# da03/torch-Attention-OCR

Measured on AMD Instinct MI355X. Metric: image-lines/sec (train step), higher is better.
Workload: dtype bf16; 1 GPU; c3: 32x256 crops, batch 256/GPU, VGG-7 + BiLSTM(256) + 2-layer attn decoder, L=24; global_batch=256, per_gpu_batch=256, img=32x256, decoder_steps=24, parallelism=dp1, input_feed=True

## Files before the change

### torch-attention-ocr_amd/csrc/knobs.h

```cpp
#pragma once
#include <cstdlib>

namespace aocr { namespace knob {
#define AOCR_KNOB_SET(FN, NAME, DEF)  inline bool FN() { return std::getenv(NAME) != nullptr; }
#define AOCR_KNOB_ON(FN, NAME, DEF)   inline bool FN() { const char* e = std::getenv(NAME); return e && e[0] == '1'; }
#define AOCR_KNOB_NOT0(FN, NAME, DEF) inline bool FN() { const char* e = std::getenv(NAME); return !(e && e[0] == '0'); }
#define AOCR_KNOB_INT(FN, NAME, DEF)  inline int FN() { const char* e = std::getenv(NAME); return e ? std::atoi(e) : (DEF); }
#define AOCR_KNOB_RAW(FN, NAME, DEF)  inline const char* FN() { return std::getenv(NAME); }
#define KNOB(NAME, KIND, DEF, EFFECT) AOCR_KNOB_##KIND(NAME, #NAME, DEF)
#define KNOB_CLAMP(NAME, KIND, DEF, LO, HI, EFFECT) inline int NAME() { const char* e = std::getenv(#NAME); if (!e) return (DEF); const int n = std::atoi(e); return n < (LO) ? (LO) : n > (HI) ? (HI) : n; }
#define KNOB_ALSO(FN, NAME, KIND, DEF, EFFECT) AOCR_KNOB_##KIND(FN, #NAME, DEF)

KNOB(AOCR_TRACE,                 SET,  0,    "one stderr line per launch decision of the traced launchers")
KNOB(AOCR_PROBE,                 SET,  0,    "aocr_profile_kernel prints the in-kernel clock probe of the tagged conv launch")
KNOB(AOCR_PROBE_LAYER,           RAW,  0,    "3|4|5: aocr_profile_kernel id 0 replays that conv layer's tagged forward launch instead of conv6's")
KNOB(AOCR_DBG_STOP,              INT,  0,    "1|2: stop the CNN backward pass at that stage and leave its gradient map in place (tap g0)")
KNOB_ALSO(AOCR_DBG_STOP_SET, AOCR_DBG_STOP, SET, 0, "cnn_wgrad_on_side: any value keeps the CNN filter gradients off the side stream")
KNOB(AOCR_DC_STAMPS,             RAW,  0,    "cycle stamps of the decoder cluster / chain kernels (stamps build); a value starting with b: beam launches only")
KNOB(AOCR_SEQ_STAMP,             SET,  0,    "cycle stamps of the whole-sequence encoder forward kernel")
KNOB(AOCR_SEQ_ABL,               INT,  0,    "timing-only ablation bits of the whole-sequence encoder forward kernel")
KNOB(AOCR_CL_REMOTE,             SET,  0,    "cluster kernels exchange through write-through stores as if their members were not on one XCD")
KNOB(AOCR_NO_DMA,                ON,   0,    "no LDS-DMA kernels at all (the 128 x 128 LDS kernels)")
KNOB(AOCR_FORCE_DMA,             ON,   0,    "LDS-DMA kernels wherever their shape constraints hold, however the grid fills the chip")
KNOB(AOCR_NO_HALO,               ON,   0,    "no halo-resident 3 x 3 kernel (the im2col LDS-DMA kernel)")
KNOB(AOCR_HALO8,                 SET,  0,    "the 8-wave gemm_halo_bf16_kernel instead of the 4-wave gemm_halo4_bf16_kernel")
KNOB(AOCR_HALO4_STAGED,          INT,  7,    "bits: output tiles of the 256 x 256 kernels through LDS -- 1 fp32 data gradient, 2 fp32 conv forward, 4 pooled")
KNOB(AOCR_NO_NARROW_WIDE,        SET,  0,    "conv7 forward on 128 x 128 tiles instead of 256 x 128 tiles of the narrow LDS-DMA kernel")
KNOB(AOCR_NO_NARROW_STAGED,      ON,   0,    "quad epilogue of the narrow LDS-DMA kernel instead of the staged tile")
KNOB(AOCR_NO_DMA128,             ON,   0,    "128 x 128 tiles on the register-staged kernel instead of gemm_dma128_kernel")
KNOB(AOCR_DMA128_W4,             ON,   0,    "gemm_dma128_kernel's 4-wave form at every grid size")
KNOB(AOCR_NO_HH_NARROW,          SET,  0,    "hoisted bf16 GEMMs on the 128 x 128 kernels instead of the narrow LDS-DMA kernel")
KNOB(AOCR_HH_NARROW_FULL_ONLY,   ON,   0,    "hoisted GEMMs take the narrow LDS-DMA kernel only when M is whole 256-row tiles")
KNOB(AOCR_NO_HH_CAT,             ON,   0,    "the encoder's d X as two products instead of one over the concatenated K range")
KNOB(AOCR_NO_SKINNY,             SET,  0,    "128 x 128 tiles for skinny products (N <= 64) instead of the step kernel; also turns project_loss_kernel off")
KNOB(AOCR_NO_PROJ_FUSE,          ON,   0,    "projector, criterion and projector data gradient as three launches instead of project_loss_kernel")
KNOB(AOCR_NO_BN_STATS_FUSE,      SET,  0,    "BatchNorm statistics of conv3 / conv5 by a pass over y instead of from the conv epilogue")
KNOB(AOCR_BN_Y16,                SET,  0,    "pre-BatchNorm maps stored as bf16 (outside the parity tolerance)")
KNOB(AOCR_DX16,                  ON,   0,    "bf16 data-gradient maps for the BatchNorm backward / un-pool passes (outside the parity tolerance)")
KNOB(AOCR_BNB_FUSE,              ON,   0,    "BatchNorm backward's sums pass from the data gradient's staged fp32 tile (measured slower)")
KNOB(AOCR_WGRAD_ATOMIC,          SET,  0,    "split-K filter gradients through fp32 atomics instead of slabs + splitk_reduce_kernel")
KNOB(AOCR_NO_WGRAD_HALO,         ON,   0,    "filter gradients on the one-tap-per-tile kernels instead of conv_wgrad_halo_kernel")
KNOB(AOCR_WGRAD_HALO_MINN,       INT,  576,  "smallest N = 9 Cin that takes conv_wgrad_halo_kernel (conv2 upwards)")
KNOB(AOCR_WGRAD_HALO_MINSTEPS,   INT,  0,    "> 0: at small P fewer, longer k ranges of at least n steps instead of a full round of the chip")
KNOB(AOCR_WGRAD_HALO_RAGGED,     NOT0, 1,    "0: conv_wgrad_halo_kernel only for rows of whole 32-pixel segments")
KNOB(AOCR_NO_WGRAD_ISSUE_MID,    ON,   0,    "conv_wgrad_halo_kernel issues the next DMA pieces before its first MFMA instead of between the k-halves")
KNOB(AOCR_NO_WGRAD_DMA_GROUPED,  ON,   0,    "recurrent weight gradients on wgrad_tr_grouped_kernel instead of wgrad_dma_grouped_kernel")
KNOB(AOCR_WGRAD_DMA_WGS,         INT,  256,  "workgroups wgrad_dma_grouped_kernel aims at per launch (one round)")
KNOB(AOCR_WGRAD_DMA_MINK,        INT,  2048, "smallest K (rows L B / T B) that takes wgrad_dma_grouped_kernel")
KNOB(AOCR_NO_LDS_F32,            SET,  0,    "fragment-from-global fp32 GEMM instead of the LDS-tiled kernels")
KNOB(AOCR_NO_F32T,               ON,   0,    "gemm_lds_f32_kernel instead of gemm_f32t_kernel")
KNOB(AOCR_F32T_TILE,             INT,  0,    "1|2|3: force gemm_f32t_kernel's tile (128 x 128 / 64 x 128 / 64 x 64)")
KNOB(AOCR_NO_F32W,               ON,   0,    "fragment-from-global kernel instead of gemm_f32w_kernel")
KNOB_CLAMP(AOCR_F32W_MINK,       INT,  192,  32, 0x7fffffff, "least K per k range of gemm_f32w_kernel's split (at least 32)")
KNOB(AOCR_NO_STEP_F32,           ON,   0,    "gemm_small_kernel<false> instead of gemm_step_f32_kernel")
KNOB(AOCR_STEP_F32_W16,          ON,   0,    "gemm_step_f32_kernel's 16-wave form for deep K on small grids (measured slower)")
KNOB(AOCR_NO_QUARTER_TILES,      SET,  0,    "full gate tiles instead of 8-unit tiles at small batch (fp32 mode)")
KNOB(AOCR_NO_HALF_TILES,         ON,   0,    "32-unit gate tiles instead of half gate tiles on small grids")
KNOB(AOCR_HALF_TILES_MAXGRID,    INT,  200,  "the 32-unit grid size below which gate products take half tiles")
KNOB(AOCR_STEP_WAVES4,           SET,  0,    "4-wave gemm_step_kernel instead of 8 waves")
KNOB(AOCR_STEP_WAVES16,          SET,  0,    "16 waves for plain step products at K >= 1024 (measured slower)")
KNOB(AOCR_NO_STEP_MT2,           ON,   0,    "one 32-row tile per workgroup instead of two where the grid allows")
KNOB(AOCR_STEP_MT2_MINK,         INT,  2048, "the K from which one plain product takes two row tiles per workgroup")
KNOB(AOCR_NO_STEPL,              ON,   0,    "step products on gemm_step_kernel instead of stepl.h")
KNOB(AOCR_STEPL_MIN_WGS,         INT,  -1,   ">= 0: stepl.h from n of its own workgroups whatever the kind of launch")
KNOB(AOCR_BIG_STEP,              ON,   0,    "step products as 128 x 128 LDS-DMA tiles + an elementwise cell pass (measured slower)")
KNOB(AOCR_BIG_STEP_MIN_ROWS,     INT,  320,  "rows from which AOCR_BIG_STEP applies")
KNOB(AOCR_CONV1_SCALAR,          SET,  0,    "conv1's filter gradient on the scalar kernel instead of the packed one")
KNOB(AOCR_UNPOOL4,               SET,  0,    "un-pool on the 4-channel kernels instead of unpool8_kernel")
KNOB(AOCR_BN_PARTIAL_OLD,        SET,  0,    "4-byte-access BatchNorm partial sums instead of bn_partial4_kernel")
KNOB(AOCR_ATTN_BWD_TWO_PASS,     SET,  0,    "the streamed attention backward kernel in two passes over the context instead of one")
KNOB(AOCR_NO_ATTN_BF16,          SET,  0,    "fp32-context attention instead of the bf16-context kernels")
KNOB(AOCR_NO_ATTN_BEAM_GROUP,    SET,  0,    "beam decode at T > 64 with one attention workgroup per hypothesis instead of per image")
KNOB(AOCR_ATTN_NW16,             SET,  0,    "16-wave attention at T <= 32, Hd = 1024")
KNOB(AOCR_NO_CHAIN_CTXA,         SET,  0,    "the Hd = 1024 chain with a q = W_a h launch per step instead of scores against ctx W_a")
KNOB(AOCR_NO_BN_FOLD,            SET,  0,    "unfused evaluation-mode BatchNorm")
KNOB(AOCR_NO_SIDE_WGRAD,         SET,  0,    "no side stream: weight gradients on the main stream")
KNOB(AOCR_SIDE_PLAIN,            SET,  0,    "side stream at normal priority")
KNOB(AOCR_NO_SIDE_PROLOGUE,      ON,   0,    "gradient zeroing / weight shadows / token table on the main stream in front of conv1")
KNOB(AOCR_NO_SHADOW_SPLIT,       ON,   0,    "conv2 waits for the whole shadow table instead of its own taps")
KNOB(AOCR_NO_CNN_WGRAD_SIDE,     ON,   0,    "the CNN's filter gradients on the main stream")
KNOB(AOCR_CNN_WGRAD_AFTER_DGRAD, ON,   0,    "filter gradient of a stage started behind its data gradient (slower)")
KNOB(AOCR_NO_COLSUM_DEFER,       SET,  0,    "one column-sum launch per bias instead of two deferred ones")
KNOB(AOCR_CONV1_RECOMPUTE,       SET,  0,    "conv1's filter gradient re-evaluates the layer instead of reading the forward pass's routes")
KNOB(AOCR_NO_SEQ,                ON,   0,    "encoder: no whole-sequence kernels at all (per-step launches)")
KNOB(AOCR_NO_CLUSTER,            ON,   0,    "encoder: no cluster kernels (one-workgroup-per-16-rows whole-sequence kernels)")
KNOB(AOCR_NO_LAYER_PIPE,         SET,  0,    "stacked encoder layer after layer instead of the chunk wavefront")
KNOB(AOCR_LAYER_PIPE_CHUNKS,     RAW,  0,    "n: force the wavefront's chunk count")
KNOB(AOCR_ENC_DC_COPY,           ON,   0,    "split copy of the decoder's initial-state gradient in front of the encoder BPTT")
KNOB(AOCR_NO_ENC_WGRAD_SIDE,     ON,   0,    "the encoder's weight gradients on the main stream")
KNOB(AOCR_SIDE_GO_LATE,          ON,   0,    "side streams released behind d(context) instead of behind the decoder BPTT")
KNOB(AOCR_NO_SIDE2,              ON,   0,    "no second side stream")
KNOB(AOCR_JOIN_BEFORE_CNN_BWD,   ON,   0,    "the main stream joins the side stream in front of the CNN backward pass")
KNOB(AOCR_NO_Q_SIDE,             ON,   0,    "q of all steps on the main stream")
KNOB(AOCR_NO_EMB_TABLE,          ON,   0,    "first decoder layer's embedding part as a gathered tensor + product instead of the per-token table")
KNOB(AOCR_NO_EMB_TABLE_CHAIN,    ON,   0,    "the launch chain's first decoder layer without the per-token table")
KNOB(AOCR_NO_DEC_CLUSTER,        ON,   0,    "decoder: launch chain instead of the cluster kernels")
KNOB(AOCR_NO_DEC_CLUSTER_BWD,    ON,   0,    "decoder BPTT: launch chain instead of the cluster kernel")
KNOB(AOCR_NO_DEC_CLUSTER_DROP,   SET,  0,    "decoder under dropout: launch chain instead of the cluster kernels")
KNOB(AOCR_NO_DEC_GREEDY,         SET,  0,    "greedy decode on the launch chain instead of the cluster kernel")
KNOB(AOCR_NO_DECODE_SHADOWS,     ON,   0,    "the decode launch chain without bf16 shadows of its beam state")
KNOB(AOCR_NO_DEC_CHAINS,         ON,   0,    "dec_cluster.hip's one-chain kernels instead of dec_chain.hip")
KNOB(AOCR_NO_DEC_CHAINS_BWD,     SET,  0,    "the same for the decoder BPTT only")
KNOB(AOCR_NO_DEC_CHAINS_GREEDY,  SET,  0,    "the same for greedy decode only")
KNOB(AOCR_NO_DEC_CHAINS_BEAM,    SET,  0,    "beam search on the per-step launch chain")
KNOB(AOCR_CH_NO_RES,             SET,  0,    "the ctx W_a tile re-read per step instead of resident (T <= 64)")
KNOB(AOCR_NO_DEC_EARLY,          SET,  0,    "no early exit of the greedy kernel")
KNOB(AOCR_ENC_RT2,               ON,   0,    "two row tiles per encoder group although one fits the chip")
KNOB(AOCR_ENC_RH16,              ON,   0,    "encoder forward on 16-row groups")
KNOB(AOCR_ENC_BWD_RH,            RAW,  0,    "8|16: force 8- / 16-row groups in the encoder BPTT")
KNOB(AOCR_ONE_COMM,              SET,  0,    "SyncBN on the gradient communicator (no ncclCommSplit)")
KNOB(AOCR_COMM_EARLY_BUCKET0,    ON,   0,    "release gradient bucket 0 before the encoder BPTT")
KNOB_CLAMP(AOCR_COMM_RESERVE_CUS, INT, 32,   0, 128, "compute units the encoder cluster launches then leave to the collective (0..128)")

#undef KNOB_ALSO
#undef KNOB_CLAMP
#undef KNOB
#undef AOCR_KNOB_RAW
#undef AOCR_KNOB_INT
#undef AOCR_KNOB_NOT0
#undef AOCR_KNOB_ON
#undef AOCR_KNOB_SET

}}
```

### torch-attention-ocr_amd/csrc/mfma_gemm.h

```cpp
#pragma once
#include <hip/hip_runtime.h>
#include <stdint.h>
#include <type_traits>
#include <utility>

namespace aocr {

typedef float f32x16 __attribute__((ext_vector_type(16)));
typedef float f32x4 __attribute__((ext_vector_type(4)));
typedef __bf16 bf16x8 __attribute__((ext_vector_type(8)));

template <int NV> struct Frag { float v[NV]; };

template <bool BF16> struct Mode {
  static constexpr int NV = BF16 ? 8 : 4;
  static constexpr int CHUNK = BF16 ? 16 : 8;
};


struct LoadK {
  const float* p0; int64_t ld0; int K0;
  const float* p1; int64_t ld1;
  int rows; int K; int vec;
  struct Ctx { const float* b0; const float* b1; bool ok; };
// ... 1946 lines not shown
#pragma unroll
  for (int i = 0; i < 4; ++i)
#pragma unroll
    for (int j = 0; j < 2; ++j)
#pragma unroll
      for (int e = 0; e < 16; ++e) acc[i][j][e] = 0.f;

  const int g = lane >> 4, q = (lane >> 2) & 3, p4 = lane & 3;
  const unsigned rowoff = (8 * h + q) * 512 + (16 * (g & 1) + 4 * p4) * 2;
  unsigned aseg[4], bseg[2];
#pragma unroll
  for (int i = 0; i < 4; ++i) aseg[i] = rowoff + (((wm * 4 + i) ^ q) << 6);
#pragma unroll
  for (int i = 0; i < 2; ++i) bseg[i] = 16384 + rowoff + (((wn * 2 + i) ^ q) << 6);

  typedef unsigned long long u64;
  typedef u64 u64x2 __attribute__((ext_vector_type(2)));
  const unsigned lbase = (unsigned)(uintptr_t)((__attribute__((address_space(3))) unsigned char*)lds);
#define AOCR_TRR(dst, addr, OFF) asm volatile("ds_read_b64_tr_b16 %0, %1 offset:" #OFF : "=v"(dst) : "v"(addr))
#pragma unroll
  for (int t = 0; t < 3; ++t) issue();
  for (int kt = 0; kt < nk; ++kt) {
    asm volatile("s_waitcnt vmcnt(8)" ::: "memory");
    __builtin_amdgcn_s_barrier();
    const unsigned sl = lbase + (kt & 3) * 32768;
    u64 fa[2][4][2], fb[2][2][2];
#pragma unroll
    for (int i = 0; i < 4; ++i) {
      const unsigned ad = sl + aseg[i];
      if constexpr (ABL & 4) { fa[0][i][0] = fa[0][i][1] = fa[1][i][0] = fa[1][i][1] = ad; continue; }
      AOCR_TRR(fa[0][i][0], ad, 0); AOCR_TRR(fa[0][i][1], ad, 2048); AOCR_TRR(fa[1][i][0], ad, 8192); AOCR_TRR(fa[1][i][1], ad, 10240);
    }
#pragma unroll
    for (int i = 0; i < 2; ++i) {
      const unsigned ad = sl + bseg[i];
      if constexpr (ABL & 4) { fb[0][i][0] = fb[0][i][1] = fb[1][i][0] = fb[1][i][1] = ad; continue; }
      AOCR_TRR(fb[0][i][0], ad, 0); AOCR_TRR(fb[0][i][1], ad, 2048); AOCR_TRR(fb[1][i][0], ad, 8192); AOCR_TRR(fb[1][i][1], ad, 10240);
    }
    if constexpr (!(ABL & 1)) issue();
    asm volatile("s_waitcnt lgkmcnt(0)"
                 : "+v"(fa[0][0][0]), "+v"(fa[0][0][1]), "+v"(fa[0][1][0]), "+v"(fa[0][1][1]), "+v"(fa[0][2][0]), "+v"(fa[0][2][1]),
                   "+v"(fa[0][3][0]), "+v"(fa[0][3][1]), "+v"(fb[0][0][0]), "+v"(fb[0][0][1]), "+v"(fb[0][1][0]), "+v"(fb[0][1][1])
                 :: "memory");
    asm volatile(""
                 : "+v"(fa[1][0][0]), "+v"(fa[1][0][1]), "+v"(fa[1][1][0]), "+v"(fa[1][1][1]), "+v"(fa[1][2][0]), "+v"(fa[1][2][1]),
                   "+v"(fa[1][3][0]), "+v"(fa[1][3][1]), "+v"(fb[1][0][0]), "+v"(fb[1][0][1]), "+v"(fb[1][1][0]), "+v"(fb[1][1][1])
                 :: "memory");
#pragma unroll
    for (int s2 = 0; s2 < 2; ++s2)
#pragma unroll
      for (int mi = 0; mi < 4; ++mi)
#pragma unroll
        for (int ni = 0; ni < 2; ++ni) {
          const u64x2 av = {fa[s2][mi][0], fa[s2][mi][1]}, bv = {fb[s2][ni][0], fb[s2][ni][1]};
          if constexpr (ABL & 2) { acc[mi][ni][0] += (float)(unsigned)(av[0] ^ bv[1]); continue; }
          acc[mi][ni] = __builtin_amdgcn_mfma_f32_32x32x16_bf16(__builtin_bit_cast(bf16x8, av), __builtin_bit_cast(bf16x8, bv), acc[mi][ni], 0, 0, 0);
        }
  }
#undef AOCR_TRR
  asm volatile("s_waitcnt vmcnt(0) lgkmcnt(0)" ::: "memory");
  const int r = lane & 31;
  const int m0 = m_blk + wm * 128, n0 = n_blk + wn * 64;
  if constexpr (std::is_same<EP, EpStore>::value && ABL == 0) {
    if (part && !ep.flags && !ep.bias && !ep.bias2 && !ep.C1 && !ep.Cb && !ep.dg && m_blk + 256 <= ep.M && n_blk + 256 <= ep.N) {
      tile256_store_f32<2, 512>(ep.C, ep.ldc, nullptr, false, acc, lds, m_blk, n_blk, wm, wn, r, h, tid);
      return;
    }
  }
#pragma unroll
  for (int mi = 0; mi < 4; ++mi)
#pragma unroll
    for (int qq = 0; qq < 4; ++qq) {
      float v[2][4];
#pragma unroll
      for (int ni = 0; ni < 2; ++ni)
#pragma unroll
        for (int i = 0; i < 4; ++i) v[ni][i] = acc[mi][ni][4 * qq + i];
      ep.template quad<2>(m0 + 32 * mi + 8 * qq + 4 * h, n0 + r, 32, v);
    }
}

struct WgDmaProblem { const bf16_t* A; const bf16_t* B; long long lda, ldb; int M, N, K, gx, tiles, ks, kper, first; float* part; float* C; long long ldc; long long f4first; };
struct WgDmaArgs { int n, total; long long f4total; WgDmaProblem p[8]; };
template <int UNUSED = 0>
__global__ __launch_bounds__(512, 1) void wgrad_dma_grouped_kernel(WgDmaArgs g, const bf16_t* zero) {
  __shared__ __attribute__((aligned(1024))) unsigned char lds[4 * 32768];
  int pi = 0;
#pragma unroll
  for (int i = 1; i < 8; ++i) if (i < g.n && (int)blockIdx.x >= g.p[i].first) pi = i;
  const WgDmaProblem& P = g.p[pi];
  const int local = blockIdx.x - P.first;
  const int zsp = local / P.tiles, bid = local - zsp * P.tiles;
  const int m_blk = (bid / P.gx) * 256, n_blk = (bid % P.gx) * 256;
  const int kbeg = zsp * P.kper, kend = min(P.K, kbeg + P.kper);
  const int nk = kend > kbeg ? (kend - kbeg + 31) >> 5 : 0;
  const int tid = threadIdx.x, lane = tid & 63, wave = __builtin_amdgcn_readfirstlane(tid >> 6);
  const int h = lane >> 5, wm = wave >> 2, wn = wave & 3;
  const bf16_t* pa[2]; const bf16_t* pb[2]; int ka[2];
#pragma unroll
  for (int j = 0; j < 2; ++j) {
    const int krow = 2 * (2 * wave + j) + (lane >> 5), pos = lane & 31;
    const int chunk = ((((pos >> 2) ^ (krow & 3)) << 2) | (pos & 3));
    ka[j] = kbeg + krow;
    pa[j] = P.A + (long long)ka[j] * P.lda + m_blk + 8 * chunk; pb[j] = P.B + (long long)ka[j] * P.ldb + n_blk + 8 * chunk;
  }
  const long long astep = 32 * P.lda, bstep = 32 * P.ldb;
  unsigned char* const wbase = lds + (2 * wave) * 1024;
  int slot = 0;
  auto issue = [&]() {
#pragma unroll
    for (int j = 0; j < 2; ++j) { dma16(dma_select(ka[j] < kend, pa[j], zero), wbase + slot * 32768 + j * 1024); pa[j] += astep; }
#pragma unroll
    for (int j = 0; j < 2; ++j) { dma16(dma_select(ka[j] < kend, pb[j], zero), wbase + slot * 32768 + 16384 + j * 1024); pb[j] += bstep; ka[j] += 32; }
    slot = (slot + 1) & 3;
  };
  f32x16 acc[4][2];
#pragma unroll
  for (int i = 0; i < 4; ++i)
#pragma unroll
    for (int j = 0; j < 2; ++j)
#pragma unroll
      for (int e = 0; e < 16; ++e) acc[i][j][e] = 0.f;
  const int gq = lane >> 4, q = (lane >> 2) & 3, p4 = lane & 3;
  const unsigned rowoff = (8 * h + q) * 512 + (16 * (gq & 1) + 4 * p4) * 2;
  unsigned aseg[4], bseg[2];
#pragma unroll
  for (int i = 0; i < 4; ++i) aseg[i] = rowoff + (((wm * 4 + i) ^ q) << 6);
#pragma unroll
  for (int i = 0; i < 2; ++i) bseg[i] = 16384 + rowoff + (((wn * 2 + i) ^ q) << 6);
  typedef unsigned long long u64;
  typedef u64 u64x2 __attribute__((ext_vector_type(2)));
  const unsigned lbase = (unsigned)(uintptr_t)((__attribute__((address_space(3))) unsigned char*)lds);
#define AOCR_TRR(dst, addr, OFF) asm volatile("ds_read_b64_tr_b16 %0, %1 offset:" #OFF : "=v"(dst) : "v"(addr))
#pragma unroll
  for (int t = 0; t < 3; ++t) issue();
  for (int kt = 0; kt < nk; ++kt) {
    asm volatile("s_waitcnt vmcnt(8)" ::: "memory");
    __builtin_amdgcn_s_barrier();
    const unsigned sl = lbase + (kt & 3) * 32768;
    u64 fa[2][4][2], fb[2][2][2];
#pragma unroll
    for (int i = 0; i < 4; ++i) {
      const unsigned ad = sl + aseg[i];
      AOCR_TRR(fa[0][i][0], ad, 0); AOCR_TRR(fa[0][i][1], ad, 2048); AOCR_TRR(fa[1][i][0], ad, 8192); AOCR_TRR(fa[1][i][1], ad, 10240);
    }
#pragma unroll
    for (int i = 0; i < 2; ++i) {
      const unsigned ad = sl + bseg[i];
      AOCR_TRR(fb[0][i][0], ad, 0); AOCR_TRR(fb[0][i][1], ad, 2048); AOCR_TRR(fb[1][i][0], ad, 8192); AOCR_TRR(fb[1][i][1], ad, 10240);
    }
    issue();
    asm volatile("s_waitcnt lgkmcnt(0)"
                 : "+v"(fa[0][0][0]), "+v"(fa[0][0][1]), "+v"(fa[0][1][0]), "+v"(fa[0][1][1]), "+v"(fa[0][2][0]), "+v"(fa[0][2][1]),
                   "+v"(fa[0][3][0]), "+v"(fa[0][3][1]), "+v"(fb[0][0][0]), "+v"(fb[0][0][1]), "+v"(fb[0][1][0]), "+v"(fb[0][1][1])
                 :: "memory");
    asm volatile(""
                 : "+v"(fa[1][0][0]), "+v"(fa[1][0][1]), "+v"(fa[1][1][0]), "+v"(fa[1][1][1]), "+v"(fa[1][2][0]), "+v"(fa[1][2][1]),
                   "+v"(fa[1][3][0]), "+v"(fa[1][3][1]), "+v"(fb[1][0][0]), "+v"(fb[1][0][1]), "+v"(fb[1][1][0]), "+v"(fb[1][1][1])
                 :: "memory");
#pragma unroll
    for (int s2 = 0; s2 < 2; ++s2)
#pragma unroll
      for (int mi = 0; mi < 4; ++mi)
#pragma unroll
        for (int ni = 0; ni < 2; ++ni) {
          const u64x2 av = {fa[s2][mi][0], fa[s2][mi][1]}, bv = {fb[s2][ni][0], fb[s2][ni][1]};
          acc[mi][ni] = __builtin_amdgcn_mfma_f32_32x32x16_bf16(__builtin_bit_cast(bf16x8, av), __builtin_bit_cast(bf16x8, bv), acc[mi][ni], 0, 0, 0);
        }
  }
#undef AOCR_TRR
  asm volatile("s_waitcnt vmcnt(0) lgkmcnt(0)" ::: "memory");
  tile256_store_f32<2, 512>(P.part + (size_t)zsp * P.M * P.N, P.N, nullptr, false, acc, lds, m_blk, n_blk, wm, wn, lane & 31, h, tid);
}
template <int UNUSED = 0>
__global__ __launch_bounds__(256) void wgrad_slab_reduce_kernel(WgDmaArgs g) {
  typedef float f4 __attribute__((ext_vector_type(4)));
  const long long i = (long long)blockIdx.x * 256 + threadIdx.x;
  if (i >= g.f4total) return;
  int pi = 0;
#pragma unroll
  for (int k = 1; k < 8; ++k) if (k < g.n && i >= g.p[k].f4first) pi = k;
  const WgDmaProblem& P = g.p[pi];
  const long long li = i - P.f4first; const int n4 = P.N >> 2; const long long m = li / n4; const int c = (int)(li - m * n4) * 4;
  const size_t mn = (size_t)P.M * P.N;
  const float* src = P.part + (size_t)m * P.N + c;
  f4 acc = {0.f, 0.f, 0.f, 0.f};
  for (int z = 0; z < P.ks; ++z) acc += __builtin_nontemporal_load(reinterpret_cast<const f4*>(src + (size_t)z * mn));
  float* o = P.C + m * P.ldc + c;
  o[0] += acc[0]; o[1] += acc[1]; o[2] += acc[2]; o[3] += acc[3];
}

template <int... I, class F> __device__ __forceinline__ void aocr_static_for_impl(std::integer_sequence<int, I...>, F&& f) { (f(std::integral_constant<int, I>{}), ...); }
template <int N, class F> __device__ __forceinline__ void aocr_static_for(F&& f) { aocr_static_for_impl(std::make_integer_sequence<int, N>{}, f); }
template <int TAG = 0, int MG = 4, bool RG = false, bool IM = false>
__global__ __launch_bounds__(128 * MG, 1)
void conv_wgrad_halo_kernel(const bf16_t* __restrict__ dy, const bf16_t* __restrict__ x, float* __restrict__ part, long long pstride,
                            int nimg, int H, int W, int Cin, int Cout, int gx, int gy, int gz, int segs_per, const bf16_t* zero) {
  constexpr int MT = 64 * MG, NWV = 2 * MG, AROW = MT * 2, RPP = 1024 / AROW, LPR = 64 / RPP;
  constexpr int BOFF = 32 * AROW, SLOT = BOFF + 8192, NS = 6, PW = 34, HPW = 8 / NWV;
  __shared__ __attribute__((aligned(1024))) unsigned char lds[NWV * 20480 > NS * SLOT ? NWV * 20480 : NS * SLOT];
  const int nwg = gx * gy * gz, orig = blockIdx.x;
  const int q8 = nwg >> 3, r8 = nwg & 7, xcd = orig & 7;
  const int lin = (xcd < r8 ? xcd * (q8 + 1) : r8 * (q8 + 1) + (xcd - r8) * q8) + (orig >> 3);
  const int zsp = lin / (gx * gy), bid = lin - zsp * (gx * gy);
  const int m_blk = (bid / gx) * MT, cchunk = bid % gx;
  const int spr = (W + 31) >> 5, S = nimg * H * spr;
  const int s_beg = zsp * segs_per, s_end = min(S, s_beg + segs_per);
  const int nk = s_end > s_beg ? s_end - s_beg : 0;
  const int tid = threadIdx.x, lane = tid & 63, wave = __builtin_amdgcn_readfirstlane(tid >> 6);
  const int h = lane >> 5, mg = wave & (MG - 1), tg = wave / MG;

  const int wrap_px = W - 32 * (spr - 1);
  const int64_t seg0_px = (int64_t)(s_beg / spr) * W + 32 * (s_beg % spr);
  const bf16_t* pa[2]; int akrow[2];
#pragma unroll
  for (int j = 0; j < 2; ++j) {
    const int krow = RPP * (2 * wave + j) + lane / LPR, pos = lane & (LPR - 1);
    const int chunk = ((((pos >> 2) ^ (krow & 3)) << 2) | (pos & 3));
    akrow[j] = krow;
    pa[j] = dy + (seg0_px + krow) * Cout + m_blk + 8 * chunk;
  }
  const int64_t astep = (int64_t)32 * Cout, awrap = (int64_t)wrap_px * Cout;
  bool bin[HPW]; int bry[HPW], bcx[HPW]; const bf16_t* pb[HPW];
#pragma unroll
  for (int j = 0; j < HPW; ++j) {
    const int sl = 64 * (HPW * wave + j) + lane;
    bin[j] = sl < 3 * PW * 4;
    const int hry = sl / (PW * 4), hrem = sl - hry * (PW * 4), hcx = hrem >> 2, hc = hrem & 3;
    bry[j] = hry - 1; bcx[j] = hcx - 1;
    pb[j] = x + (seg0_px + (int64_t)(hry - 1) * W + (hcx - 1)) * Cin + cchunk * 32 + hc * 8;
  }
  const int64_t bstep = (int64_t)32 * Cin, bwrap = (int64_t)wrap_px * Cin;
  int is = s_beg, ixs = s_beg % spr, iy = (s_beg / spr) % H;
  unsigned char* const wA = lds + (2 * wave) * 1024;
  unsigned char* const wB = lds + BOFF + (HPW * wave) * 1024;
  int islot = 0;
  auto issue = [&]() {
    const bool live = is < s_end;
    const int x0 = ixs << 5;
    if constexpr (RG) {
      const bool last = ixs + 1 == spr;
#pragma unroll
      for (int j = 0; j < 2; ++j) { dma16(dma_select(live && x0 + akrow[j] < W, pa[j], zero), wA + islot * SLOT + j * 1024); pa[j] += last ? awrap : astep; }
#pragma unroll
      for (int j = 0; j < HPW; ++j) {
        const bool ok = live && bin[j] && (unsigned)(iy + bry[j]) < (unsigned)H && (unsigned)(x0 + bcx[j]) < (unsigned)W;
        dma16(dma_select(ok, pb[j], zero), wB + islot * SLOT + j * 1024); pb[j] += last ? bwrap : bstep;
      }
      ++is; if (last) { ixs = 0; if (++iy == H) iy = 0; } else ++ixs;
    } else {
#pragma unroll
      for (int j = 0; j < 2; ++j) { dma16(dma_select(live, pa[j], zero), wA + islot * SLOT + j * 1024); pa[j] += astep; }
#pragma unroll
      for (int j = 0; j < HPW; ++j) {
        const bool ok = live && bin[j] && (unsigned)(iy + bry[j]) < (unsigned)H && (unsigned)(x0 + bcx[j]) < (unsigned)W;
// ... 487 lines not shown
```

### torch-attention-ocr_amd/csrc/ops_gemm.hip

```cpp
#include "ops.h"
#include "stepl.h"

namespace aocr {

static void split_k(int K, int chunk, int& ksplit, int& kper) {
  if (ksplit < 1) ksplit = 1;
  kper = cdiv(cdiv(K, ksplit), chunk) * chunk;
  if (kper < chunk) kper = chunk;
  ksplit = cdiv(K, kper); if (ksplit < 1) ksplit = 1;
}
static thread_local const char* t_trace_fn = nullptr;
struct TraceScope { explicit TraceScope(const char* fn) { t_trace_fn = fn; } ~TraceScope() { t_trace_fn = nullptr; } };
static void trace_launch(const char* kernel, const char* inst, long long M, long long N, long long K) {
  if (t_trace_fn && knob::AOCR_TRACE()) fprintf(stderr, "[aocr] %s: %s[%s] %lld %lld %lld\n", t_trace_fn, kernel, inst, M, N, K);
}
static void trace_step(int nt, int gates, int waves, int mt, long long M, long long N, long long K) {
  if (!t_trace_fn || !knob::AOCR_TRACE()) return;
  char inst[32]; snprintf(inst, sizeof inst, "%d,%d,w%d%s", nt, gates, waves, mt == 2 ? ",mt2" : "");
  trace_launch("gemm_step_kernel", inst, M, N, K);
}
template <class AL, class BL, class EP>
static void launch_lds(hipStream_t s, const AL& a, const BL& b, const EP& ep, int M, int N, int K, int ksplit) {
  if (M <= 0 || N <= 0) return;
  int kper; split_k(K, 32, ksplit, kper);
// ... 595 lines not shown
    for (int i = 0; i < nd; ++i) hs[nh++] = ds[i];
  for (int base = 0; base < nh; base += 8)
    grouped_launch<LoadMNh>(s, hs + base, std::min(8, nh - base), 1024, true, wgrad_tr_grouped_kernel<EpStore>);
  for (int base = 0; base < nf; base += 8)
    grouped_launch<LoadMN>(s, fs + base, std::min(8, nf - base), 768, false, gemm_lds_grouped_kernel<LoadMN, LoadMN, EpStore>);
}

static LoadConvK make_convk(const float* src, int B, int Hs, int Ws, int C, int ks, int sgn, int off, int Hr, int Wr, int pool) {
  LoadConvK a; a.src = src; a.H = Hs; a.W = Ws; a.C = C; a.KW = ks; a.sgn = sgn; a.off = off; a.Hr = Hr; a.Wr = Wr;
  a.pmode = pool; a.Hp = Hr / 2; a.Wp = Wr / 2;
  if (pool == 1) a.rows = B * a.Hp * a.Wp * 4; else if (pool == 2) a.rows = B * a.Hp * Wr * 2; else a.rows = B * Hr * Wr;
  a.K = ks * ks * C;
  return a;
}

void conv_forward(hipStream_t s, bool bf16, const float* x, const float* w, const float* bias, float* y, uint8_t* idx, int B,
                  int H, int W, int Cin, int Cout, int ks, int pad, int relu, int pool, const bf16_t* xb, const bf16_t* wb,
                  bf16_t* yb, int profile_tag, const float* bn_save, const float* bn_w, const float* bn_b, double* bn_part, int* bn_chunks, int* y_bf16) {
  const TraceScope ts("conv_forward");
  const int Ho = H + 2 * pad - ks + 1, Wo = W + 2 * pad - ks + 1;
  LoadConvK a = make_convk(x, B, H, W, Cin, ks, 1, -pad, Ho, Wo, pool);
  EpConv ep; ep.y = y; ep.idx = idx; ep.bias = bias; ep.Cout = Cout; ep.rows = a.rows; ep.pmode = pool; ep.relu = relu; ep.yb = yb;
  ep.bn_save = bn_save; ep.bn_w = bn_w; ep.bn_b = bn_b;
  if (bn_chunks) *bn_chunks = 0;
  if (y_bf16) *y_bf16 = 0;
  if (bf16 && xb && wb) {
    LoadConvKh ah; ah.src = xb; ah.g = a;
    LoadKh bh; bh.p = wb; bh.ld = a.K; bh.rows = Cout; bh.K = a.K;
    if (bn_part && bn_chunks && y && !yb && !bn_save && pool == 0 && dma_eligible(a.rows, Cout, a.K, Cin) && a.rows % 256 == 0 && a.rows / 256 <= 512 && !knob::AOCR_NO_BN_STATS_FUSE()) {
      if (staged256(2, pad == 1 && halo_eligible(a, Cout, 256, 256))) {
        ep.bn_part = bn_part; *bn_chunks = a.rows / 256;
        if (y_bf16 && knob::AOCR_BN_Y16() && Cout % 4 == 0 && !knob::AOCR_BN_PARTIAL_OLD()) {
          ep.y16 = reinterpret_cast<bf16_t*>(y); ep.y = nullptr; *y_bf16 = 1; }
      }
    }
    if (dma_eligible(a.rows, Cout, a.K, Cin) && pad == 1 && halo_eligible(a, Cout, 256, 256)) launch_halo<1, 256, 256>(s, ah, bh, ep, a.rows, Cout, profile_tag);
    else if (dma_eligible(a.rows, Cout, a.K, Cin)) launch_dma(s, ah, bh, ep, a.rows, Cout, a.K, profile_tag);
    else if (dma_narrow_eligible(a.rows, Cout, a.K, Cin) || dma_mid_eligible(a.rows, Cout, a.K, Cin)) launch_dma_narrow(s, ah, bh, ep, a.rows, Cout, a.K);
    else if (dma128_eligible(a.rows, Cout, a.K, Cin)) launch_dma128(s, ah, bh, ep, a.rows, Cout, a.K);
    else launch_lds(s, ah, bh, ep, a.rows, Cout, a.K, 1);
  } else {
    launch_conv_fwd(s, bf16, a, make_loadk(w, a.K, Cout, a.K), ep, a.rows, Cout, a.K);
  }
}

static bool dgrad_bf16_out(const LoadConvK& a, int Cin, int Cout, int pad) {
  return dma_eligible(a.rows, Cin, a.K, Cout) && a.rows % 256 == 0 && Cin % 256 == 0 && knob::AOCR_DX16() && !knob::AOCR_BN_PARTIAL_OLD() && !knob::AOCR_UNPOOL4() &&
         staged256(1, pad == 1 && halo_eligible(a, Cin, 256, 256));
}
bool conv_dgrad_bf16_out(int B, int H, int W, int Cin, int Cout, int ks, int pad) {
  const int Ho = H + 2 * pad - ks + 1, Wo = W + 2 * pad - ks + 1;
  return dgrad_bf16_out(make_convk(nullptr, B, Ho, Wo, Cout, ks, -1, pad, H, W, 0), Cin, Cout, pad);
}

void conv_backward_data(hipStream_t s, bool bf16, const float* dy, const float* w, float* dx, int B, int H, int W, int Cin,
                        int Cout, int ks, int pad, const bf16_t* dyb, const bf16_t* wtb, const float* wtf, int* dx16, const BnBwdFuse* bnb, int* bnb_chunks) {
  const TraceScope ts("conv_backward_data");
  const int Ho = H + 2 * pad - ks + 1, Wo = W + 2 * pad - ks + 1;
  LoadConvK a = make_convk(dy, B, Ho, Wo, Cout, ks, -1, pad, H, W, 0);
  EpStore ep = make_store(dx, Cin, a.rows, Cin);
  if (dx16) *dx16 = 0;
  if (bnb_chunks) *bnb_chunks = 0;
  if (bf16 && dyb && wtb) {
    LoadConvKh ah; ah.src = dyb; ah.g = a;
    LoadKh bh; bh.p = wtb; bh.ld = a.K; bh.rows = Cin; bh.K = a.K;
    if (dx16 && dgrad_bf16_out(a, Cin, Cout, pad)) { ep.C = nullptr; ep.Cb = reinterpret_cast<bf16_t*>(dx); ep.ldcb = Cin; *dx16 = 1; }
    if (bnb && bnb_chunks && ep.C && dma_eligible(a.rows, Cin, a.K, Cout) && a.rows % 256 == 0 && Cin % 256 == 0 && a.rows / 256 <= 512 && knob::AOCR_BNB_FUSE() &&
        staged256(1, pad == 1 && halo_eligible(a, Cin, 256, 256))) {
      ep.bnb_x = bnb->x; ep.bnb_yb = bnb->yb; ep.bnb_save = bnb->save; ep.bnb_part = bnb->part; *bnb_chunks = a.rows / 256;
    }
    if (dma_eligible(a.rows, Cin, a.K, Cout) && pad == 1 && halo_eligible(a, Cin, 256, 256)) launch_halo<-1, 256, 256>(s, ah, bh, ep, a.rows, Cin);
    else if (dma_eligible(a.rows, Cin, a.K, Cout)) launch_dma(s, ah, bh, ep, a.rows, Cin, a.K);
    else if (dma_narrow_eligible(a.rows, Cin, a.K, Cout)) launch_dma_narrow(s, ah, bh, ep, a.rows, Cin, a.K);
    else if (dma128_eligible(a.rows, Cin, a.K, Cout)) launch_dma128(s, ah, bh, ep, a.rows, Cin, a.K);
    else launch_lds(s, ah, bh, ep, a.rows, Cin, a.K, 1);
  } else if (wtf) {
    launch_big(s, bf16, a, make_loadk(wtf, a.K, Cin, a.K), ep, a.rows, Cin, a.K, 1);
  } else {
    LoadConvWT b; b.w = w; b.Cin = Cin; b.Cout = Cout; b.KK = ks * ks; b.K = a.K;
    launch_conv_dgrad(s, bf16, a, b, ep, a.rows, Cin, a.K);
  }
}

void conv_backward_filter(hipStream_t s, bool bf16, const float* x, const float* dy, float* dw, float* dbias, int B, int H,
                          int W, int Cin, int Cout, int ks, int pad, const bf16_t* xb, const bf16_t* dyb, float* part, size_t part_floats, int profile_tag) {
  const TraceScope ts("conv_backward_filter");
  const int Ho = H + 2 * pad - ks + 1, Wo = W + 2 * pad - ks + 1;
  const int P = B * Ho * Wo, N = ks * ks * Cin;
  LoadConvXcol b; b.x = x; b.H = H; b.W = W; b.Cin = Cin; b.KW = ks; b.pad = pad; b.Ho = Ho; b.Wo = Wo; b.N = N; b.K = P;
  EpStore ep = make_store(dw, N, Cout, N, nullptr, nullptr, EP_ATOMIC);
  const int ksplit = pick_ksplit(Cout, N, P, bf16, (bf16 && xb && dyb) ? 1024 : 768);
  if (bf16 && xb && dyb) {
    LoadMNh ah; ah.p = dyb; ah.ld = Cout; ah.rows = Cout; ah.K = P;
    LoadConvXcolh bh; bh.x = xb; bh.g = b;
    const int tiles = cdiv(N, 256) * (Cout / 256);
    const int hmt = Cout % 256 == 0 ? 256 : 128;
    const int spr = (W + 31) / 32;
    const bool ragged_ok = W % 32 == 0 || (knob::AOCR_WGRAD_HALO_RAGGED() && W * 4 >= spr * 32 * 3);
    if (ks == 3 && pad == 1 && ragged_ok && Cout % hmt == 0 && Cin % 32 == 0 && part && !knob::AOCR_NO_DMA() && !knob::AOCR_NO_WGRAD_HALO() && !knob::AOCR_WGRAD_ATOMIC() &&
        (knob::AOCR_FORCE_DMA() || (P >= 8192 && N >= knob::AOCR_WGRAD_HALO_MINN()))) {
      const int htiles = (Cin / 32) * (Cout / hmt), S = B * H * spr;
      int ksh = htiles >= 256 ? 1 : 256 / htiles; if (ksh > S) ksh = S;
      { const int minsteps = knob::AOCR_WGRAD_HALO_MINSTEPS();
        if (minsteps > 0 && S / ksh < minsteps) ksh = std::max(1, S / minsteps); }
      const int per = cdiv(S, ksh); ksh = cdiv(S, per);
      const size_t mn = (size_t)Cout * N;
      if (mn * ksh <= part_floats) {
#define AOCR_WGH(TAGV, MGV, RGV, IMV, THREADS, MTV) hipLaunchKernelGGL((conv_wgrad_halo_kernel<TAGV, MGV, RGV, IMV>), dim3(htiles * ksh), dim3(THREADS), 0, s, dyb, xb, part, (long long)mn, B, H, W, Cin, Cout, Cin / 32, Cout / MTV, ksh, per, zero_page())
        const bool im = !knob::AOCR_NO_WGRAD_ISSUE_MID();
        { char inst[48]; snprintf(inst, sizeof inst, "%d,%s,%s", hmt, W % 32 ? "ragged" : "whole", im ? "issue_mid" : "no_issue_mid");
          trace_launch("conv_wgrad_halo_kernel", inst, Cout, N, P); }
        if (W % 32) {
          if (hmt == 128) { if (im) AOCR_WGH(0, 2, true, true, 256, 128); else AOCR_WGH(0, 2, true, false, 256, 128); }
          else { if (im) AOCR_WGH(0, 4, true, true, 512, 256); else AOCR_WGH(0, 4, true, false, 512, 256); }
        }
        else if (hmt == 128) { if (im) AOCR_WGH(0, 2, false, true, 256, 128); else AOCR_WGH(0, 2, false, false, 256, 128); }
        else if (profile_tag) { if (im) AOCR_WGH(1, 4, false, true, 512, 256); else AOCR_WGH(1, 4, false, false, 512, 256); }
        else { if (im) AOCR_WGH(0, 4, false, true, 512, 256); else AOCR_WGH(0, 4, false, false, 512, 256); }
#undef AOCR_WGH
        splitk_reduce(s, part, ksh, mn, dw);
        if (dbias) colsum_accum(s, dy, Cout, P, Cout, dbias);
        return;
      }
    }
    if (Cout % 256 == 0 && Cin % 8 == 0 && !knob::AOCR_NO_DMA() && (knob::AOCR_FORCE_DMA() || (P >= 8192 && tiles <= 256 && N % 256 == 0 && N >= 2304))) {
      int ks2 = tiles >= 128 ? (tiles >= 200 ? 1 : 2) : 256 / tiles, kper2; split_k(P, 32, ks2, kper2);
      const size_t mn = (size_t)Cout * N;
      float* const slab = (part && ks2 > 1 && mn * ks2 <= part_floats && !knob::AOCR_WGRAD_ATOMIC()) ? part : nullptr;
      trace_launch("conv_wgrad_dma_kernel", slab ? "slab" : "atomic", Cout, N, P);
      if (profile_tag)
        hipLaunchKernelGGL((conv_wgrad_dma_kernel<EpStore, 256>), dim3(tiles * ks2), dim3(512), 0, s, ah, bh, ep, P, kper2, cdiv(N, 256), Cout / 256, zero_page(), ks2, slab, (long long)mn);
      else
        hipLaunchKernelGGL((conv_wgrad_dma_kernel<EpStore>), dim3(tiles * ks2), dim3(512), 0, s, ah, bh, ep, P, kper2, cdiv(N, 256), Cout / 256, zero_page(), ks2, slab, (long long)mn);
      if (slab) splitk_reduce(s, slab, ks2, mn, dw);
      if (dbias) colsum_accum(s, dy, Cout, P, Cout, dbias);
      return;
    }
    int ks = ksplit, kper; split_k(P, 32, ks, kper);
    const int gx = cdiv(N, 128), gy = cdiv(Cout, 128);
    const size_t mn = (size_t)Cout * N;
    float* const slab = (part && ks > 1 && mn * ks <= part_floats && !knob::AOCR_WGRAD_ATOMIC()) ? part : nullptr;
    trace_launch("conv_wgrad_tr_kernel", slab ? "slab" : "atomic", Cout, N, P);
    hipLaunchKernelGGL((conv_wgrad_tr_kernel<EpStore>), dim3(gx * gy * ks), dim3(256), 0, s, ah, bh, ep, P, kper, gx, gy, ks, slab, (long long)mn);
    if (slab) splitk_reduce(s, slab, ks, mn, dw);
  } else {
    launch_conv_wgrad(s, bf16, make_loadmn(dy, Cout, Cout, P), b, ep, Cout, N, P, ksplit);
  }
  if (dbias) colsum_accum(s, dy, Cout, P, Cout, dbias);
}

}
```

Measured before the change: 54240 image-lines/s.

## Route conv7 filter gradient through grouped LDS-DMA wgrad kernel with image-gap addressing

Adds a conv-aware variant of wgrad_dma_grouped_kernel for the 2x2, pad-0, single-output-row conv7 layer. It treats the two kernel rows as two grouped GEMM problems whose B operand walks input pixels, skipping the gap between images. Partial slabs are interleaved so one split-K reduce writes the full filter gradient. The aim is to replace the slower one-tap-per-tile path with the DMA-fed 256x256 MFMA tiles. In exchange it adds per-step index bookkeeping and a fixed k-range count chosen by a knob.

```diff
diff --git a/torch-attention-ocr_amd/csrc/knobs.h b/torch-attention-ocr_amd/csrc/knobs.h
--- a/torch-attention-ocr_amd/csrc/knobs.h
+++ b/torch-attention-ocr_amd/csrc/knobs.h
@@ -47,6 +47,8 @@
 KNOB(AOCR_NO_WGRAD_DMA_GROUPED,  ON,   0,    "recurrent weight gradients on wgrad_tr_grouped_kernel instead of wgrad_dma_grouped_kernel")
 KNOB(AOCR_WGRAD_DMA_WGS,         INT,  256,  "workgroups wgrad_dma_grouped_kernel aims at per launch (one round)")
 KNOB(AOCR_WGRAD_DMA_MINK,        INT,  2048, "smallest K (rows L B / T B) that takes wgrad_dma_grouped_kernel")
+KNOB(AOCR_NO_CONV7_WGRAD_DMA,    ON,   0,    "conv7's filter gradient on the one-tap-per-tile kernels instead of wgrad_dma_grouped_kernel<1>")
+KNOB(AOCR_CONV7_WGRAD_RANGES,    INT,  4,    "k ranges of conv7's filter gradient on wgrad_dma_grouped_kernel<1> (16 tiles each: 4 = 64 work items)")
 KNOB(AOCR_NO_LDS_F32,            SET,  0,    "fragment-from-global fp32 GEMM instead of the LDS-tiled kernels")
 KNOB(AOCR_NO_F32T,               ON,   0,    "gemm_lds_f32_kernel instead of gemm_f32t_kernel")
 KNOB(AOCR_F32T_TILE,             INT,  0,    "1|2|3: force gemm_f32t_kernel's tile (128 x 128 / 64 x 128 / 64 x 64)")
diff --git a/torch-attention-ocr_amd/csrc/mfma_gemm.h b/torch-attention-ocr_amd/csrc/mfma_gemm.h
--- a/torch-attention-ocr_amd/csrc/mfma_gemm.h
+++ b/torch-attention-ocr_amd/csrc/mfma_gemm.h
@@ -2052,8 +2052,11 @@
 
 struct WgDmaProblem { const bf16_t* A; const bf16_t* B; long long lda, ldb; int M, N, K, gx, tiles, ks, kper, first; float* part; float* C; long long ldc; long long f4first; };
 struct WgDmaArgs { int n, total; long long f4total; WgDmaProblem p[8]; };
-template <int UNUSED = 0>
-__global__ __launch_bounds__(512, 1) void wgrad_dma_grouped_kernel(WgDmaArgs g, const bf16_t* zero) {
+struct WgDmaConvArgs : WgDmaArgs { int wo; long long gap; };
+template <int CONV> struct WgDmaArgsOf { typedef WgDmaArgs type; };
+template <> struct WgDmaArgsOf<1> { typedef WgDmaConvArgs type; };
+template <int CONV = 0>
+__global__ __launch_bounds__(512, 1) void wgrad_dma_grouped_kernel(typename WgDmaArgsOf<CONV>::type g, const bf16_t* zero) {
   __shared__ __attribute__((aligned(1024))) unsigned char lds[4 * 32768];
   int pi = 0;
 #pragma unroll
@@ -2067,12 +2070,14 @@
   const int tid = threadIdx.x, lane = tid & 63, wave = __builtin_amdgcn_readfirstlane(tid >> 6);
   const int h = lane >> 5, wm = wave >> 2, wn = wave & 3;
   const bf16_t* pa[2]; const bf16_t* pb[2]; int ka[2];
+  int xr[2];
 #pragma unroll
   for (int j = 0; j < 2; ++j) {
     const int krow = 2 * (2 * wave + j) + (lane >> 5), pos = lane & 31;
     const int chunk = ((((pos >> 2) ^ (krow & 3)) << 2) | (pos & 3));
     ka[j] = kbeg + krow;
     pa[j] = P.A + (long long)ka[j] * P.lda + m_blk + 8 * chunk; pb[j] = P.B + (long long)ka[j] * P.ldb + n_blk + 8 * chunk;
+    if constexpr (CONV) { const int img = ka[j] / g.wo; xr[j] = ka[j] - img * g.wo; pb[j] += img * g.gap; }
   }
   const long long astep = 32 * P.lda, bstep = 32 * P.ldb;
   unsigned char* const wbase = lds + (2 * wave) * 1024;
@@ -2081,7 +2086,14 @@
 #pragma unroll
     for (int j = 0; j < 2; ++j) { dma16(dma_select(ka[j] < kend, pa[j], zero), wbase + slot * 32768 + j * 1024); pa[j] += astep; }
 #pragma unroll
-    for (int j = 0; j < 2; ++j) { dma16(dma_select(ka[j] < kend, pb[j], zero), wbase + slot * 32768 + 16384 + j * 1024); pb[j] += bstep; ka[j] += 32; }
+    for (int j = 0; j < 2; ++j) {
+      dma16(dma_select(ka[j] < kend, pb[j], zero), wbase + slot * 32768 + 16384 + j * 1024); pb[j] += bstep; ka[j] += 32;
+      if constexpr (CONV) {
+        xr[j] += 32;
+        if (g.wo >= 32) { const bool w = xr[j] >= g.wo; xr[j] -= w ? g.wo : 0; pb[j] += w ? g.gap : 0; }
+        else while (xr[j] >= g.wo) { xr[j] -= g.wo; pb[j] += g.gap; }
+      }
+    }
     slot = (slot + 1) & 3;
   };
   f32x16 acc[4][2];
@@ -2140,7 +2152,10 @@
   }
 #undef AOCR_TRR
   asm volatile("s_waitcnt vmcnt(0) lgkmcnt(0)" ::: "memory");
-  tile256_store_f32<2, 512>(P.part + (size_t)zsp * P.M * P.N, P.N, nullptr, false, acc, lds, m_blk, n_blk, wm, wn, lane & 31, h, tid);
+  if constexpr (CONV)
+    tile256_store_f32<2, 512>(P.part + (size_t)zsp * 2 * P.M * P.N, 2 * P.N, nullptr, false, acc, lds, m_blk, n_blk, wm, wn, lane & 31, h, tid);
+  else
+    tile256_store_f32<2, 512>(P.part + (size_t)zsp * P.M * P.N, P.N, nullptr, false, acc, lds, m_blk, n_blk, wm, wn, lane & 31, h, tid);
 }
 template <int UNUSED = 0>
 __global__ __launch_bounds__(256) void wgrad_slab_reduce_kernel(WgDmaArgs g) {
diff --git a/torch-attention-ocr_amd/csrc/ops_gemm.hip b/torch-attention-ocr_amd/csrc/ops_gemm.hip
--- a/torch-attention-ocr_amd/csrc/ops_gemm.hip
+++ b/torch-attention-ocr_amd/csrc/ops_gemm.hip
@@ -701,6 +701,33 @@
   }
 }
 
+static bool conv7_wgrad_dma_ok(int Cin, int Cout, int ks, int pad, int Ho, int P, const float* part) {
+  return ks == 2 && pad == 0 && Ho == 1 && Cout % 256 == 0 && (2 * Cin) % 256 == 0 && part && !knob::AOCR_NO_DMA() && !knob::AOCR_WGRAD_ATOMIC() &&
+         !knob::AOCR_NO_CONV7_WGRAD_DMA() && (P >= 8192 || knob::AOCR_FORCE_DMA());
+}
+static bool conv7_wgrad_dma(hipStream_t s, const bf16_t* xb, const bf16_t* dyb, float* dw, int B, int H, int W, int Cin, int Cout, float* part, size_t part_floats) {
+  const int Wo = W - 1, P = B * Wo, N = 2 * Cin;
+  if (Wo < 1 || ((reinterpret_cast<uintptr_t>(xb) | reinterpret_cast<uintptr_t>(dyb)) & 15)) return false;
+  const int tiles = (Cout / 256) * (N / 256);
+  int ks = std::max(1, knob::AOCR_CONV7_WGRAD_RANGES()), kper; split_k(P, 32, ks, kper);
+  const size_t mn = (size_t)Cout * N;
+  while (ks > 1 && 2 * mn * ks > part_floats) { --ks; split_k(P, 32, ks, kper); }
+  if (2 * mn * ks > part_floats) return false;
+  WgDmaConvArgs g; g.n = 2; g.wo = Wo; g.gap = (long long)(H * W - Wo) * Cin;
+  for (int ky = 0; ky < 2; ++ky) {
+    WgDmaProblem& Q = g.p[ky];
+    Q.A = dyb; Q.B = xb + (size_t)ky * W * Cin; Q.lda = Cout; Q.ldb = Cin; Q.M = Cout; Q.N = N; Q.K = P;
+    Q.gx = N / 256; Q.tiles = tiles; Q.ks = ks; Q.kper = kper; Q.first = ky * tiles * ks;
+    Q.part = part + (size_t)ky * N;
+    Q.C = dw + (size_t)ky * N; Q.ldc = 2 * N; Q.f4first = 0;
+  }
+  g.total = 2 * tiles * ks; g.f4total = 0;
+  { char inst[32]; snprintf(inst, sizeof inst, "conv7,ks%d", ks); trace_launch("wgrad_dma_grouped_kernel", inst, Cout, 2 * N, P); }
+  hipLaunchKernelGGL((wgrad_dma_grouped_kernel<1>), dim3(g.total), dim3(512), 0, s, g, zero_page());
+  splitk_reduce(s, part, ks, 2 * mn, dw);
+  return true;
+}
+
 void conv_backward_filter(hipStream_t s, bool bf16, const float* x, const float* dy, float* dw, float* dbias, int B, int H,
                           int W, int Cin, int Cout, int ks, int pad, const bf16_t* xb, const bf16_t* dyb, float* part, size_t part_floats, int profile_tag) {
   const TraceScope ts("conv_backward_filter");
@@ -712,6 +739,10 @@
   if (bf16 && xb && dyb) {
     LoadMNh ah; ah.p = dyb; ah.ld = Cout; ah.rows = Cout; ah.K = P;
     LoadConvXcolh bh; bh.x = xb; bh.g = b;
+    if (conv7_wgrad_dma_ok(Cin, Cout, ks, pad, Ho, P, part) && conv7_wgrad_dma(s, xb, dyb, dw, B, H, W, Cin, Cout, part, part_floats)) {
+      if (dbias) colsum_accum(s, dy, Cout, P, Cout, dbias);
+      return;
+    }
     const int tiles = cdiv(N, 256) * (Cout / 256);
     const int hmt = Cout % 256 == 0 ? 256 : 128;
     const int spr = (W + 31) / 32;
```

New measurement: 54620 image-lines/s, median of 6. No clear change (+0.7%).
